# MDIL-SNU/SevenNet

Hardware: NVIDIA H100
Metric: atom_updates_per_sec (higher is better)
Workload: dtype f32

## Files before the change

sevenn_b200/csrc/common.cuh:

```cuda
#pragma once
#include <cuda_runtime.h>
#include <cstdint>
#include <cstdio>

#include "vec_ops.cuh"

namespace s7b {

constexpr float kSiluNorm = 1.6791767923989418f;
constexpr int kMaxPaths = 12;
constexpr int kMaxL = 4;

S7B_HD float silu_n(float z) {
  const float s = 1.0f / (1.0f + expf(-z));
  return kSiluNorm * z * s;
}
S7B_HD float dsilu_n(float z) {
  const float s = 1.0f / (1.0f + expf(-z));
  return kSiluNorm * s * (1.0f + z * (1.0f - s));
}

struct ConvRole {
  int x_off;
  int mul;
  int tab_off;
  int w_off[kMaxPaths];
  int out_off[kMaxPaths];
  int out_stride[kMaxPaths];
  int ftab_off;
};

__host__ __device__ constexpr int y_stride(int ny) { return (ny - 1 + 3) / 4 * 4; }

constexpr int kConvWrongMul = 3;
constexpr int kConvNoPath = 4;

struct ConvArgs {
  const int* rowptr;
  const int4* rec;
  const float* Y;
  const float* x;
  const float4* table;
  const uint2* table23;
  const float* w;
  int n_begin, n_dst;
  int dim_x, dim_mid, w_numel;
  float inv_h;
  unsigned int* row_max;
  int rows_per_node;
  const float2* ftable;
  float ftab_inv_h;
  int ftab_knots;
};

struct ConvTangents {
  const float* x;
  const float* Y;
  const float* w;
};

}

#define S7B_CUDA_CHECK(expr)                                                            \
  do {                                                                                  \
    cudaError_t _e = (expr);                                                            \
    if (_e != cudaSuccess) {                                                            \
      s7b::set_error(__FILE__, __LINE__, cudaGetErrorString(_e));                       \
      return 1;                                                                         \
    }                                                                                   \
  } while (0)

namespace s7b {
void set_error(const char* file, int line, const char* msg);
}
```

sevenn_b200/csrc/conv_kernels.cuh:

```cuda
#pragma once
#include <cuda_fp16.h>

#include "common.cuh"
#include "generated/tp_kinds.cuh"
#include "tp_tangent.cuh"

namespace s7b {

constexpr int kConvWarpsPerBlock = 4;
constexpr int kConvMul[kMaxL] = {128, 64, 32, 32};
constexpr int kConvMaxMul = 1024;

template <int MUL>
__device__ __forceinline__ int conv_mul(const ConvRole& role) {
  if constexpr (MUL > 0) return MUL;
  else return role.mul;
}
#ifndef S7B_FWD_MINBLOCKS
#define S7B_FWD_MINBLOCKS 1
#endif
#define S7B_FWD_BOUNDS __launch_bounds__(32 * kConvWarpsPerBlock, S7B_FWD_MINBLOCKS)
#ifdef S7B_BWD_MINBLOCKS
#define S7B_BWD_BOUNDS __launch_bounds__(32 * kConvWarpsPerBlock, S7B_BWD_MINBLOCKS)
#else
#define S7B_BWD_BOUNDS __launch_bounds__(32 * kConvWarpsPerBlock, \
    (Kind::NY != 9 || (MUL == 0 && Kind::D1 > 1)) ? 2 : ((Kind::D1 == 3 || !NEED_DX) ? 4 : 3))
#endif
#ifndef S7B_COOP_REC
#define S7B_COOP_REC 1
#endif

constexpr float kValueTableMinR = 0.6f;

enum { kRecRaw = 0, kRecValue = 1, kRecCubicShort = 2 };
template <int MODE>
__device__ __forceinline__ int4 fwd_rec(const ConvArgs& a, int4 r, bool valid, bool& short_seen) {
  const float rr = __int_as_float(r.w);
  const bool is_short = valid && rr < kValueTableMinR;
  if (MODE == kRecValue) {
    short_seen = short_seen || is_short;
    const int k = is_short ? a.ftab_knots - 1 : min(max((int)(rr * a.ftab_inv_h), 0), a.ftab_knots - 1);
    const float t = is_short ? 1.0f : fminf(fmaxf(fmaf(rr, a.ftab_inv_h, -(float)k), 0.0f), 1.0f);
    return make_int4(r.x, k, __float_as_int(t), 0);
  }
  if (MODE == kRecCubicShort) return make_int4(r.x, is_short ? r.y : ~r.y, r.z, 0);
  return r;
}

template <int LPN>
struct EdgeRecs {
  int cx, cy, cz;
  __device__ __forceinline__ void fill(const ConvArgs& a, int e0, int len, int it, int sl) {
    const int ei = it + sl;
    int4 r = make_int4(0, 0, 0, 0);
    if (ei < len) r = __ldg(a.rec + (unsigned)(e0 + ei));
    cx = r.x; cy = r.y; cz = r.z;
  }
  template <int MODE>
  __device__ __forceinline__ void fill(const ConvArgs& a, int e0, int len, int it, int sl, bool& short_seen) {
    const int ei = it + sl;
    int4 r = make_int4(0, 0, 0, 0);
    if (ei < len) r = __ldg(a.rec + (unsigned)(e0 + ei));
    r = fwd_rec<MODE>(a, r, ei < len, short_seen);
    cx = r.x; cy = r.y; cz = r.z;
  }
  __device__ __forceinline__ int4 get(int it) const {
    const int l = it % LPN;
    return make_int4(__shfl_sync(0xffffffffu, cx, l, LPN), __shfl_sync(0xffffffffu, cy, l, LPN),
                     __shfl_sync(0xffffffffu, cz, l, LPN), 0);
  }
};

template <int M, int LPN>
__device__ __forceinline__ void group_reduce_multi(float (&v)[M], int sl) {
  static_assert((M == 8 || M == 16) && (LPN == 16 || LPN == 32) && M <= LPN, "unsupported reduction shape");
  int off = LPN / 2;
#pragma unroll
  for (int m = M / 2; m >= 1; m >>= 1, off >>= 1) {
    const bool up = (sl & off) != 0;
#pragma unroll
    for (int j = 0; j < m; ++j) {
      const float send = up ? v[j] : v[j + m];
      const float keep = up ? v[j + m] : v[j];
      v[j] = keep + __shfl_xor_sync(0xffffffffu, send, off);
    }
  }
#pragma unroll
  for (; off >= 1; off >>= 1) v[0] += __shfl_xor_sync(0xffffffffu, v[0], off);
}

template <int LPN>
__device__ __forceinline__ float group_sum(float v) {
#pragma unroll
  for (int off = LPN / 2; off >= 1; off >>= 1) v += __shfl_xor_sync(0xffffffffu, v, off);
  return v;
}

template <class Kind>
__device__ __forceinline__ void load_Y(const float* __restrict__ Yrow, float (&Y)[Kind::NY]) {
  Y[0] = 1.0f;
  constexpr int NQ = (Kind::NY - 1 + 3) / 4;
  const float4* p = reinterpret_cast<const float4*>(Yrow);
#pragma unroll
  for (int q = 0; q < NQ; ++q) {
    const float4 v = __ldg(p + q);
    if (4 * q + 1 < Kind::NY) Y[4 * q + 1] = v.x;
    if (4 * q + 2 < Kind::NY) Y[4 * q + 2] = v.y;
    if (4 * q + 3 < Kind::NY) Y[4 * q + 3] = v.z;
    if (4 * q + 4 < Kind::NY) Y[4 * q + 4] = v.w;
  }
}

__device__ __forceinline__ size_t row_offset(int i, int stride) { return (size_t)(unsigned)i * (unsigned)stride; }

__device__ __forceinline__ float2 ldg2(const float* p) { return __ldg(reinterpret_cast<const float2*>(p)); }

template <class V> struct VT;
template <> struct VT<V2> {
  static constexpr int CH = 2;
  static __device__ __forceinline__ V2 zero() { return splat2(0.0f); }
  static __device__ __forceinline__ V2 load(const float* p) { return ldg2(p); }
  static __device__ __forceinline__ void store(float* p, V2 v) { *reinterpret_cast<float2*>(p) = v; }
// ... 13 lines not shown
  static constexpr int CH = 1;
  static __device__ __forceinline__ float zero() { return 0.0f; }
  static __device__ __forceinline__ float load(const float* p) { return __ldg(p); }
  static __device__ __forceinline__ void store(float* p, float v) { *p = v; }
  static __device__ __forceinline__ float hsum(float v) { return v; }
  static __device__ __forceinline__ float amax(float v) { return fabsf(v); }
  static __device__ __forceinline__ float val(const float2* p, bool odd) { return __ldg(reinterpret_cast<const float*>(p) + odd); }
  static __device__ __forceinline__ void coef(const float4* t01, const uint2* t23, bool odd, float& a0, float& a1, float& a2, float& a3) {
    const float4 c01 = __ldg(t01);
    const uint2 c23 = __ldg(t23);
    const float2 h2 = __half22float2(*reinterpret_cast<const __half2*>(&c23.x));
    const float2 h3 = __half22float2(*reinterpret_cast<const __half2*>(&c23.y));
    a0 = odd ? c01.y : c01.x;
    a1 = odd ? c01.w : c01.z;
    a2 = odd ? h2.y : h2.x;
    a3 = odd ? h3.y : h3.x;
  }
};

template <int NV, int LPN, int CH>
struct LaneMap {
  int n, sl, uc0, e0, len, nmax;
  bool node_ok;
  __device__ __forceinline__ LaneMap(const ConvArgs& a) {
    constexpr int GPW = 32 / LPN;
    const int lane = threadIdx.x & 31;
    sl = lane % LPN;
    n = a.n_begin + (blockIdx.x * kConvWarpsPerBlock + (threadIdx.x >> 5)) * GPW + lane / LPN;
    node_ok = n < a.n_dst;
    uc0 = blockIdx.y * (CH * LPN * NV) + CH * sl;
    e0 = 0;
    len = 0;
    if (node_ok) {
      e0 = __ldg(a.rowptr + n);
      len = __ldg(a.rowptr + n + 1) - e0;
    }
    nmax = len;
    if (GPW > 1) nmax = max(len, __shfl_xor_sync(0xffffffffu, len, 16));
  }
};

template <class Kind, int MUL, int NV, int LPN, bool TABLE, class V, int MODE>
__device__ __forceinline__ void conv_fwd_edges(const ConvArgs& a, const ConvRole& role,
                                               const LaneMap<NV, LPN, VT<V>::CH>& m,
                                               V (&acc)[NV][Kind::NACC], bool& short_seen) {
  constexpr int CH = VT<V>::CH;
  const int mul = conv_mul<MUL>(role);
  const unsigned xlane = role.x_off + m.uc0;
  const unsigned tlane = (MODE == kRecCubicShort ? role.tab_off : role.ftab_off) + (m.uc0 >> 1);
  const bool odd = (m.uc0 & 1) != 0;
  EdgeRecs<LPN> recs;
  for (int it = 0; it < m.nmax; ++it) {
    const bool valid = (LPN == 32) || (it < m.len);
    const int e = valid ? m.e0 + it : 0;
#if S7B_COOP_REC
    if (it % LPN == 0) recs.template fill<MODE>(a, m.e0, m.len, it, m.sl, short_seen);
    const int4 rec = recs.get(it);
#else
    const int4 rec = fwd_rec<MODE>(a, __ldg(a.rec + e), valid, short_seen);
#endif
    float Y[Kind::NY];
    load_Y<Kind>(a.Y + row_offset(e, y_stride(Kind::NY)), Y);
    const float* __restrict__ xrow = a.x + (row_offset(rec.x, a.dim_x) + xlane);
    const bool take = MODE != kRecCubicShort || rec.y >= 0;
    const int k = take ? rec.y : ~rec.y;
    const unsigned ti = tlane + k * (Kind::NPATH * mul / 2);
    const float2* __restrict__ v0 = a.ftable + ti;
    const float2* __restrict__ v1 = v0 + Kind::NPATH * mul / 2;
    const float tt = __int_as_float(rec.z);
#pragma unroll
    for (int c = 0; c < NV; ++c) {
      const int u = CH * LPN * c;
      V x[Kind::D1], w[Kind::NPATH];
#pragma unroll
      for (int i = 0; i < Kind::D1; ++i) x[i] = VT<V>::load(xrow + i * mul + u);
#pragma unroll
      for (int p = 0; p < Kind::NPATH; ++p) {
        if (MODE == kRecValue) {
          const V w0 = VT<V>::val(v0 + (p * (mul / 2) + u / 2), odd);
          const V w1 = VT<V>::val(v1 + (p * (mul / 2) + u / 2), odd);
          w[p] = fma_(tt, w1, fma_(-tt, w0, w0));
        } else if (MODE == kRecCubicShort) {
          V a0, a1, a2, a3;
          VT<V>::coef(a.table + ti + (p * (mul / 2) + u / 2), a.table23 + ti + (p * (mul / 2) + u / 2), odd, a0, a1, a2, a3);
          w[p] = take ? fma_(tt, fma_(tt, fma_(tt, a3, a2), a1), a0) : VT<V>::zero();
        } else {
          w[p] = VT<V>::load(a.w + (size_t)e * a.w_numel + role.w_off[p] + m.uc0 + u);
        }
        if (LPN != 32 && !valid) w[p] = VT<V>::zero();
      }
      Kind::fwd(x, Y, w, acc[c]);
    }
  }
}

template <class Kind, int MUL, int NV, int LPN, bool TABLE, class V>
__global__ void S7B_FWD_BOUNDS
conv_fwd_kernel(const ConvArgs a, const ConvRole role, float* __restrict__ out) {
  constexpr int CH = VT<V>::CH;
  static_assert(MUL % (CH * LPN * NV) == 0, "channels must fill whole lane groups");
  const LaneMap<NV, LPN, CH> m(a);
  if (m.nmax == 0 && !m.node_ok) return;

  V acc[NV][Kind::NACC];
#pragma unroll
  for (int c = 0; c < NV; ++c)
#pragma unroll
    for (int q = 0; q < Kind::NACC; ++q) acc[c][q] = VT<V>::zero();

  bool short_seen = false;
  conv_fwd_edges<Kind, MUL, NV, LPN, TABLE, V, TABLE ? kRecValue : kRecRaw>(a, role, m, acc, short_seen);
// ... 22 lines not shown
      }
    }
  }
  if (!m.node_ok) return;
  float* __restrict__ orow = out + (size_t)m.n * a.dim_mid;
#pragma unroll
  for (int c = 0; c < NV; ++c) {
    const int u = m.uc0 + CH * LPN * c;
#pragma unroll
    for (int p = 0; p < Kind::NPATH; ++p) {
#pragma unroll
      for (int k = 0; k < 2 * Kind::path_l3(p) + 1; ++k)
        VT<V>::store(orow + role.out_off[p] + k * role.out_stride[p] + u, acc[c][Kind::acc_off(p) + k]);
    }
  }
}

template <class Kind, int MUL, int NV, int LPN, bool TABLE, bool NEED_DX>
__global__ void S7B_BWD_BOUNDS
conv_bwd_kernel(const ConvArgs a, const ConvRole role, const float* __restrict__ gout,
                float* __restrict__ dx, float* __restrict__ dY_acc, float* __restrict__ dEdr_acc,
                float* __restrict__ dw) {
  static_assert(MUL % (2 * LPN * NV) == 0, "channels must fill whole lane groups");
  const int mul = conv_mul<MUL>(role);
  const bool SPLIT = (MUL > 0) ? (MUL > 2 * LPN * NV) : (gridDim.y > 1);
  const LaneMap<NV, LPN, 2> m(a);
  if (m.nmax == 0) return;

  V2 ga[NV][Kind::NACC];
  {
    const float* __restrict__ grow = gout + (size_t)(m.node_ok ? m.n : 0) * a.dim_mid;
#pragma unroll
    for (int c = 0; c < NV; ++c) {
      const int u = m.uc0 + 2 * LPN * c;
#pragma unroll
      for (int p = 0; p < Kind::NPATH; ++p)
#pragma unroll
        for (int k = 0; k < 2 * Kind::path_l3(p) + 1; ++k)
          ga[c][Kind::acc_off(p) + k] = ldg2(grow + role.out_off[p] + k * role.out_stride[p] + u);
    }
  }

  constexpr int NR = (Kind::NY <= 9) ? 8 : 16;
  constexpr bool RIDE = TABLE && (Kind::NY - 1 < NR);
  constexpr int PER = LPN / NR;
  const int idx = (m.sl / PER) % NR;
  const bool is_dY = idx + 1 < Kind::NY;
  const bool writer = (m.sl % PER) == 0 && (is_dY || (RIDE && idx == NR - 1));
  const unsigned xlane = role.x_off + m.uc0;
  const unsigned tlane = role.tab_off + (m.uc0 >> 1);
  EdgeRecs<LPN> recs;
  for (int it = 0; it < m.nmax; ++it) {
    const bool valid = (LPN == 32) || (it < m.len);
    const int e = valid ? m.e0 + it : 0;
#if S7B_COOP_REC
    if (it % LPN == 0) recs.fill(a, m.e0, m.len, it, m.sl);
    const int4 rec = recs.get(it);
#else
    const int4 rec = __ldg(a.rec + e);
#endif
    float Y[Kind::NY];
    load_Y<Kind>(a.Y + row_offset(e, y_stride(Kind::NY)), Y);
    const size_t xo = row_offset(rec.x, a.dim_x) + xlane;
    const unsigned ti = tlane + rec.y * (Kind::NPATH * mul / 2);
    const float4* __restrict__ k01 = a.table + ti;
    const uint2* __restrict__ k23 = a.table23 + ti;
    const float tt = __int_as_float(rec.z);
    V2 dY[Kind::NY];
#pragma unroll
    for (int j = 0; j < Kind::NY; ++j) dY[j] = splat2(0.0f);
    V2 dEdr2 = splat2(0.0f);
#pragma unroll
    for (int c = 0; c < NV; ++c) {
      const int u = 2 * LPN * c;
      V2 x[Kind::D1], w[Kind::NPATH], wd[Kind::NPATH], dwv[Kind::NPATH], dxv[Kind::D1];
#pragma unroll
      for (int i = 0; i < Kind::D1; ++i) x[i] = ldg2(a.x + xo + (i * mul + u));
#pragma unroll
      for (int p = 0; p < Kind::NPATH; ++p) {
        if (TABLE) {
          const float4 c01 = __ldg(k01 + (p * (mul / 2) + u / 2));
          const uint2 c23 = __ldg(k23 + (p * (mul / 2) + u / 2));
          const V2 a0 = make_float2(c01.x, c01.y), a1 = make_float2(c01.z, c01.w);
          const V2 a2 = __half22float2(*reinterpret_cast<const __half2*>(&c23.x));
          const V2 a3 = __half22float2(*reinterpret_cast<const __half2*>(&c23.y));
          w[p] = fma_(tt, fma_(tt, fma_(tt, a3, a2), a1), a0);
          wd[p] = mul_(fma_(tt, fma_(3.0f * tt, a3, mul_(a2, 2.0f)), a1), a.inv_h);
        } else {
          w[p] = ldg2(a.w + (size_t)e * a.w_numel + role.w_off[p] + m.uc0 + u);
        }
      }
      Kind::bwd(x, Y, w, ga[c], dwv, dxv, dY);
      if (valid) {
#pragma unroll
        for (int p = 0; p < Kind::NPATH; ++p) {
          if (TABLE) dEdr2 = fma_(dwv[p], wd[p], dEdr2);
          else *reinterpret_cast<float2*>(dw + (size_t)e * a.w_numel + role.w_off[p] + m.uc0 + u) = dwv[p];
        }
        if (NEED_DX) {
#pragma unroll
          for (int i = 0; i < Kind::D1; ++i)
            atomicAdd(reinterpret_cast<float2*>(dx + xo + (i * mul + u)), dxv[i]);
        }
      }
    }
    const float dEdr = dEdr2.x + dEdr2.y;
    float red[NR];
#pragma unroll
    for (int j = 0; j < NR; ++j) red[j] = (j + 1 < Kind::NY) ? dY[j + 1].x + dY[j + 1].y : 0.0f;
    if (RIDE) red[NR - 1] = dEdr;
    group_reduce_multi<NR, LPN>(red, m.sl);
    if (valid && writer) {
      float* dst = is_dY ? dY_acc + row_offset(e, y_stride(Kind::NY)) + idx : dEdr_acc + e;
      if (SPLIT) atomicAdd(dst, red[0]);
      else *dst += red[0];
    }
    if (TABLE && !RIDE) {
      const float s = group_sum<LPN>(dEdr);
      if (valid && m.sl == 0) {
        if (SPLIT) atomicAdd(dEdr_acc + e, s);
        else dEdr_acc[e] += s;
      }
    }
  }
}

template <class Kind, int NV, int LPN>
__global__ void S7B_FWD_BOUNDS
conv_jvp_kernel(const ConvArgs a, const ConvRole role, const ConvTangents tan, float* __restrict__ out) {
  const LaneMap<NV, LPN, 2> m(a);
  if (m.nmax == 0 && !m.node_ok) return;
  const int mul = role.mul;
  const bool hx = tan.x != nullptr, hY = tan.Y != nullptr, hw = tan.w != nullptr;

  V2 acc[NV][Kind::NACC];
#pragma unroll
  for (int c = 0; c < NV; ++c)
#pragma unroll
    for (int q = 0; q < Kind::NACC; ++q) acc[c][q] = splat2(0.0f);

  const unsigned xlane = role.x_off + m.uc0;
  EdgeRecs<LPN> recs;
  for (int it = 0; it < m.nmax; ++it) {
    const bool valid = (LPN == 32) || (it < m.len);
    const int e = valid ? m.e0 + it : 0;
    if (it % LPN == 0) recs.fill(a, m.e0, m.len, it, m.sl);
    const int4 rec = recs.get(it);
    float Y[Kind::NY], tY[Kind::NY];
    load_Y<Kind>(a.Y + row_offset(e, y_stride(Kind::NY)), Y);
    if (hY) load_Y<Kind>(tan.Y + row_offset(e, y_stride(Kind::NY)), tY);
    const size_t xo = row_offset(rec.x, a.dim_x) + xlane;
    const size_t wo = (size_t)e * a.w_numel + m.uc0;
#pragma unroll
    for (int c = 0; c < NV; ++c) {
      const int u = 2 * LPN * c;
      V2 x[Kind::D1], tx[Kind::D1], w[Kind::NPATH], tw[Kind::NPATH];
#pragma unroll
      for (int i = 0; i < Kind::D1; ++i) {
        x[i] = ldg2(a.x + xo + (i * mul + u));
        if (hx) tx[i] = ldg2(tan.x + xo + (i * mul + u));
      }
#pragma unroll
      for (int p = 0; p < Kind::NPATH; ++p) {
        w[p] = ldg2(a.w + wo + (role.w_off[p] + u));
        if (hw) tw[p] = ldg2(tan.w + wo + (role.w_off[p] + u));
        if (LPN != 32 && !valid) w[p] = tw[p] = splat2(0.0f);
      }
      TPTangent<Kind>::jvp(x, Y, w, tx, tY, tw, hx, hY, hw, acc[c]);
    }
  }
  if (!m.node_ok) return;
  float* __restrict__ orow = out + (size_t)m.n * a.dim_mid;
#pragma unroll
  for (int c = 0; c < NV; ++c) {
    const int u = m.uc0 + 2 * LPN * c;
#pragma unroll
    for (int p = 0; p < Kind::NPATH; ++p) {
#pragma unroll
      for (int k = 0; k < 2 * Kind::path_l3(p) + 1; ++k)
        VT<V2>::store(orow + role.out_off[p] + k * role.out_stride[p] + u, acc[c][Kind::acc_off(p) + k]);
    }
  }
}

enum { kTanDw = 1, kTanDx = 2, kTanDY = 4 };
template <class Kind, int NV, int LPN, int OUT>
__device__ __forceinline__ void conv_bwd_tangent_edges(const ConvArgs& a, const ConvRole& role, const ConvTangents& tan,
                                                       const LaneMap<NV, LPN, 2>& m, const V2 (&ga)[NV][Kind::NACC],
                                                       float* __restrict__ dx, float* __restrict__ dY_acc,
                                                       float* __restrict__ dw) {
  constexpr bool DW = (OUT & kTanDw) != 0, DX = (OUT & kTanDx) != 0, DY = (OUT & kTanDY) != 0;
  const int mul = role.mul;
  const bool SPLIT = gridDim.y > 1;
  const bool hx = tan.x != nullptr, hY = tan.Y != nullptr, hw = tan.w != nullptr;
  const bool need_dx = DX && (hY || hw);
  constexpr int NR = (Kind::NY <= 9) ? 8 : 16;
  constexpr int PER = LPN / NR;
  const int idx = (m.sl / PER) % NR;
  const bool writer = (m.sl % PER) == 0 && idx + 1 < Kind::NY;
  const unsigned xlane = role.x_off + m.uc0;
  EdgeRecs<LPN> recs;
  for (int it = 0; it < m.nmax; ++it) {
    const bool valid = (LPN == 32) || (it < m.len);
    const int e = valid ? m.e0 + it : 0;
    if (it % LPN == 0) recs.fill(a, m.e0, m.len, it, m.sl);
    const int4 rec = recs.get(it);
    float Y[Kind::NY], tY[Kind::NY];
    load_Y<Kind>(a.Y + row_offset(e, y_stride(Kind::NY)), Y);
    if (hY && (DW || DX)) load_Y<Kind>(tan.Y + row_offset(e, y_stride(Kind::NY)), tY);
    const size_t xo = row_offset(rec.x, a.dim_x) + xlane;
    const size_t wo = (size_t)e * a.w_numel + m.uc0;
    V2 dY[Kind::NY];
#pragma unroll
    for (int j = 0; j < Kind::NY; ++j) dY[j] = splat2(0.0f);
#pragma unroll
    for (int c = 0; c < NV; ++c) {
      const int u = 2 * LPN * c;
      V2 x[Kind::D1], tx[Kind::D1], w[Kind::NPATH], tw[Kind::NPATH], dwv[Kind::NPATH], dxv[Kind::D1];
#pragma unroll
      for (int i = 0; i < Kind::D1; ++i) {
        x[i] = ldg2(a.x + xo + (i * mul + u));
        if (hx && (DW || DY)) tx[i] = ldg2(tan.x + xo + (i * mul + u));
      }
#pragma unroll
      for (int p = 0; p < Kind::NPATH; ++p) {
        w[p] = ldg2(a.w + wo + (role.w_off[p] + u));
        if (hw && (DX || DY)) tw[p] = ldg2(tan.w + wo + (role.w_off[p] + u));
      }
      TPTangent<Kind>::template bwd<DW, DX, DY>(x, Y, w, ga[c], tx, tY, tw, hx, hY, hw, dwv, dxv, dY);
      if (valid) {
        if (DW) {
#pragma unroll
          for (int p = 0; p < Kind::NPATH; ++p)
            *reinterpret_cast<float2*>(dw + wo + (role.w_off[p] + u)) = dwv[p];
        }
        if (need_dx) {
#pragma unroll
          for (int i = 0; i < Kind::D1; ++i)
            atomicAdd(reinterpret_cast<float2*>(dx + xo + (i * mul + u)), dxv[i]);
        }
      }
    }
    if (DY) {
      float red[NR];
#pragma unroll
      for (int j = 0; j < NR; ++j) red[j] = (j + 1 < Kind::NY) ? dY[j + 1].x + dY[j + 1].y : 0.0f;
      group_reduce_multi<NR, LPN>(red, m.sl);
      if (valid && writer) {
        float* dst = dY_acc + row_offset(e, y_stride(Kind::NY)) + idx;
        if (SPLIT) atomicAdd(dst, red[0]);
        else *dst += red[0];
      }
    }
  }
}

template <class Kind>
constexpr bool tangent_walk_per_output() { return Kind::NACC * (Kind::D1 + Kind::NY) > 400; }

// ... 31 lines not shown
```

sevenn_b200/csrc/edge_kernels.cuh:

```cuda
#pragma once
#include "common.cuh"
#include "generated/sh.cuh"

namespace s7b {

struct RadialDesc {
  float cutoff;
  int cutoff_fn;
  float cutoff_on;
  int poly_p;
  int n_basis;
  float coeffs[8];
  float inv_h;
  int knots;
};

S7B_HD void envelope(const RadialDesc& d, float r, float& env, float& denv) {
  if (d.cutoff_fn == 0) {
    if (r < d.cutoff_on) { env = 1.0f; denv = 0.0f; return; }
    const float r2 = r * r, on2 = d.cutoff_on * d.cutoff_on, c2 = d.cutoff * d.cutoff;
    const float den = (c2 - on2) * (c2 - on2) * (c2 - on2);
    const float a = c2 - r2, b = c2 + 2.0f * r2 - 3.0f * on2;
    env = a * a * b / den;
    denv = (-4.0f * r * a * b + 4.0f * r * a * a) / den;
  } else {
    const float p = (float)d.poly_p;
    const float x = r / d.cutoff;
    float xp = 1.0f;
    for (int i = 0; i < d.poly_p - 1; ++i) xp *= x;
    const float c0 = (p + 1.0f) * (p + 2.0f) * 0.5f, c1 = p * (p + 2.0f), c2 = p * (p + 1.0f) * 0.5f;
    env = 1.0f - xp * x * (c0 - c1 * x + c2 * x * x);
    denv = -xp * (c0 * p - c1 * (p + 1.0f) * x + c2 * (p + 2.0f) * x * x) / d.cutoff;
  }
}

template <int LMAX>
__global__ void edge_fwd_kernel(const RadialDesc rd, const float* __restrict__ edge_vec,
                                const int* __restrict__ src, const int64_t* __restrict__ n_edges_p, int ny_stride,
                                int4* __restrict__ rec, float* __restrict__ Yout,
                                float* __restrict__ rlen, float* __restrict__ emb) {
  const int64_t e = (int64_t)blockIdx.x * blockDim.x + threadIdx.x;
  if (e >= *n_edges_p) return;
  const float vx = edge_vec[3 * e], vy = edge_vec[3 * e + 1], vz = edge_vec[3 * e + 2];
  const float r = sqrtf(vx * vx + vy * vy + vz * vz);
  const float ir = r > 0.0f ? 1.0f / r : 0.0f;
  float Y[SH<LMAX>::NY];
  SH<LMAX>::eval(vx * ir, vy * ir, vz * ir, Y);
  float* yrow = Yout + e * ny_stride;
#pragma unroll
  for (int j = 1; j < SH<LMAX>::NY; ++j) yrow[j - 1] = Y[j];
  for (int j = SH<LMAX>::NY - 1; j < ny_stride; ++j) yrow[j] = 0.0f;
  const float s = r * rd.inv_h;
  int tk = (int)s;
  tk = tk < 0 ? 0 : (tk > rd.knots - 1 ? rd.knots - 1 : tk);
  const float tt = fminf(fmaxf(s - (float)tk, 0.0f), 1.0f);
  rec[e] = make_int4(__ldg(src + e), tk, __float_as_int(tt), __float_as_int(r));
  rlen[e] = r;
  if (emb != nullptr) {
    float env, denv;
    envelope(rd, r, env, denv);
    const float pre = 2.0f / rd.cutoff;
    for (int b = 0; b < rd.n_basis; ++b) emb[e * rd.n_basis + b] = pre * sinf(rd.coeffs[b] * r) * ir * env;
  }
}

template <int LMAX>
__global__ void edge_bwd_kernel(const RadialDesc rd, const float* __restrict__ edge_vec,
                                const int64_t* __restrict__ n_edges_p, int64_t part_stride, int ny_stride, int n_part,
// ... 94 lines not shown
```

sevenn_b200/csrc/engine.cu:

```cuda
#include <algorithm>
#include <cstdlib>
#include <cstring>
#include <functional>
#include <map>
#include <string>
#include <vector>

#include "../../include/sevenn_b200.h"
#include "common.cuh"
#include "conv_kernels.cuh"
#include "edge_kernels.cuh"
#include "hvp_kernels.cuh"
#include "neighbor.cuh"
#include "node_kernels.cuh"
#include "tc_gemm.cuh"

namespace s7b {

static thread_local std::string g_error;
static int64_t g_launches = 0;
extern int64_t g_conv_launches;

void set_error(const char* file, int line, const char* msg) {
  char buf[512];
// ... 137 lines not shown
struct LayerParams {
  NodeLinear si1, si1T, sc, scT, si2, si2T;
  DevBuf table, table23, table_fwd;
  int ftab_knots = 0;
  DevBuf mlp[3], mlpT[3];
  void release() {
    for (NodeLinear* s : {&si1, &si1T, &sc, &scT, &si2, &si2T})
      for (DevBuf* b : {&s->w, &s->tc.q, &s->tc.fb}) b->release();
    for (DevBuf* b : {&table, &table23, &table_fwd, &mlp[0], &mlp[1], &mlp[2], &mlpT[0], &mlpT[1], &mlpT[2]}) b->release();
  }
};

struct HvpBufs {
  DevBuf dvec, dr, dY, gY, dgY, ar, dar, fneg, virial;
  DevBuf emb3, hA, hB, w3, dw, aw, daw1, daw2;
  DevBuf ah, dah, ag, dag, amid, damid, dmid, ax, dax, th;
  DevBuf atom_ptr1, sys_energy, dvir2;
  std::vector<DevBuf> tx, tg;
  RowExp re;
  void release() {
    for (DevBuf* b : {&dvec, &dr, &dY, &gY, &dgY, &ar, &dar, &fneg, &virial, &emb3, &hA, &hB, &w3, &dw, &aw, &daw1, &daw2,
                      &ah, &dah, &ag, &dag, &amid, &damid, &dmid, &ax, &dax, &th, &atom_ptr1, &sys_energy, &dvir2, &re.buf})
      b->release();
    for (auto* v : {&tx, &tg})
      for (DevBuf& b : *v) b.release();
  }
};

struct GlobalParams {
  DevBuf embed_x0, embed_g0, readout, readout_lo, scale, shift;
  void release() {
    for (DevBuf* b : {&embed_x0, &embed_g0, &readout, &readout_lo, &scale, &shift}) b->release();
  }
};

}

using namespace s7b;

struct S7bEngine {
  S7bModelDesc desc;
  std::vector<LayerCfg> layers;
  std::vector<LayerParams> layer_params;
  GlobalParams global_params;
  RadialDesc radial;
  bool radial_ready = false;
  int ny_stride = 8;
  int n_nodes = 0, n_local = 0, n_interior = 0;
  int64_t n_edges = 0;
  const int* d_species = nullptr;
  const int* d_rowptr = nullptr;
  const int* d_src = nullptr;
  const float* d_edge_vec = nullptr;
  DevBuf rec, Y, rlen, emb, dY_acc, dEdr_acc, demb_acc, fedge;
  std::vector<DevBuf> x, g, wbuf, z1, z2, h1, h2;
  DevBuf mid, h, dh, dg, dx, dwbuf, tmpA, tmpB;
  RowExp re_mid, re_h, re_dg, re_dx;
  DevBuf energy, atomic_energy, atomic_energy64, forces, virial, atomic_virial;
  bool want_atomic_virial = false;
  DevBuf hs_species, hs_rowptr, hs_src, hs_vec, hs_centre, hs_flag;
  DevBuf nl_pos, nl_wrapped, nl_key, nl_key_sorted, nl_idx, nl_idx_sorted, nl_bin_start, nl_count, nl_tmp, nl_centres;
  DevBuf nl_species, nl_grids, nl_atom_ptr, nl_bin_off, nl_lohi, nl_sys, nl_total;
  std::vector<NLGrid> nl_grids_host;
  std::vector<int> nl_bin_off_host;
  int nl_n_centres = 0;
  int64_t nl_n_edges = 0;
  int n_systems = 0;
  bool species_sc = false;
  DevBuf seg_perm, seg;
  DevBuf sys_atom_ptr;
  Profiler prof;
  cudaStream_t side[kMaxL] = {nullptr, nullptr, nullptr, nullptr};
  cudaEvent_t ev_fork = nullptr, ev_join[kMaxL] = {nullptr, nullptr, nullptr, nullptr};
  bool concurrent = true;
  int64_t E_cap = 0;
  DevBuf d_nE;
  cudaGraphExec_t gexec = nullptr;
  cudaStream_t gstream = nullptr;
  cudaEvent_t g_in = nullptr, g_out = nullptr;
  std::vector<int64_t> g_key;
  int64_t g_launches_per_replay = 0;
  int64_t g_captures = 0, g_replays = 0;
  struct StageGraph {
    cudaGraphExec_t exec = nullptr;
    std::vector<int64_t> key;
    int64_t launches = 0, replays_since_capture = 0;
    int thrash = 0;
  };
  std::map<int, StageGraph> stage_graphs;
  bool capturing = false;
  int64_t sg_captures = 0, sg_replays = 0;
  bool hvp_ready = false;
  HvpBufs hv;
};

struct S7bConvPlan {
  LayerCfg cfg;
  int lmax_filter = 0;
  int ny_stride = 8;
};

namespace s7b {

static int irreps_dim(const int* muls, int n_l) {
  int d = 0;
  for (int l = 0; l < n_l; ++l) d += (2 * l + 1) * muls[l];
  return d;
// ... 682 lines not shown
    P.si2 = {&L.mid, &L.g, L.g.n_l};
    P.si2T = {&L.g, &L.mid, L.g.n_l};
  }
  e->ny_stride = y_stride((d->lmax_filter + 1) * (d->lmax_filter + 1));
  e->x.resize(T);
  e->g.resize(T);
  e->wbuf.resize(T);
  e->z1.resize(T);
  e->z2.resize(T);
  e->h1.resize(T);
  e->h2.resize(T);
  memset(&e->radial, 0, sizeof(e->radial));
  e->radial.cutoff = d->cutoff;
  e->radial.cutoff_fn = d->cutoff_fn;
  e->radial.cutoff_on = d->cutoff_on;
  e->radial.poly_p = d->poly_p;
  e->radial.n_basis = d->n_basis;
  e->radial.knots = d->table_knots > 0 ? d->table_knots : 1;
  e->radial.inv_h = d->table_knots > 0 ? (float)d->table_knots / d->cutoff : 1.0f;
  e->want_atomic_virial = g_opt_atomic_virial != 0;
  for (int i = 1; i < kMaxL; ++i) {
    if (cudaStreamCreateWithFlags(&e->side[i], cudaStreamNonBlocking) != cudaSuccess ||
        cudaEventCreateWithFlags(&e->ev_join[i], cudaEventDisableTiming) != cudaSuccess) {
      delete e;
      return fail("cannot create side streams");
    }
  }
  if (cudaEventCreateWithFlags(&e->ev_fork, cudaEventDisableTiming) != cudaSuccess) {
    delete e;
    return fail("cannot create events");
  }
  *out = e;
  return 0;
}

void s7b_engine_destroy(S7bEngine* e) {
  if (!e) return;
  for (int i = 1; i < kMaxL; ++i) {
    if (e->side[i]) cudaStreamDestroy(e->side[i]);
    if (e->ev_join[i]) cudaEventDestroy(e->ev_join[i]);
  }
  if (e->ev_fork) cudaEventDestroy(e->ev_fork);
  if (e->gexec) cudaGraphExecDestroy(e->gexec);
  for (auto& kv : e->stage_graphs) if (kv.second.exec) cudaGraphExecDestroy(kv.second.exec);
  if (e->gstream) cudaStreamDestroy(e->gstream);
  if (e->g_in) cudaEventDestroy(e->g_in);
  if (e->g_out) cudaEventDestroy(e->g_out);
  e->d_nE.release();
  e->global_params.release();
  for (LayerParams& P : e->layer_params) P.release();
  for (RowExp* r : {&e->re_mid, &e->re_h, &e->re_dg, &e->re_dx}) r->buf.release();
  e->seg_perm.release();
  e->seg.release();
  DevBuf* bufs[] = {&e->rec, &e->Y, &e->rlen, &e->emb, &e->dY_acc, &e->dEdr_acc, &e->demb_acc, &e->fedge,
                    &e->mid, &e->h, &e->dh, &e->dg, &e->dx, &e->dwbuf, &e->tmpA, &e->tmpB, &e->energy,
                    &e->atomic_energy, &e->forces, &e->virial, &e->atomic_virial, &e->hs_species, &e->hs_rowptr, &e->hs_src,
                    &e->hs_vec, &e->hs_centre, &e->hs_flag, &e->nl_pos, &e->nl_wrapped, &e->nl_key, &e->nl_key_sorted,
                    &e->nl_idx, &e->nl_idx_sorted, &e->nl_bin_start, &e->nl_count, &e->nl_tmp, &e->nl_centres,
                    &e->nl_species, &e->nl_grids, &e->nl_atom_ptr, &e->nl_bin_off, &e->nl_lohi, &e->nl_sys, &e->nl_total,
                    &e->sys_atom_ptr, &e->atomic_energy64};
  for (DevBuf* b : bufs) b->release();
  for (auto* v : {&e->x, &e->g, &e->wbuf, &e->z1, &e->z2, &e->h1, &e->h2})
    for (auto& b : *v) b.release();
  e->hv.release();
  delete e;
}

int s7b_engine_set_atomic_virial(S7bEngine* e, int enable) {
  if (!e) return fail("null engine");
  if (e->want_atomic_virial != (enable != 0)) ++g_alloc_gen;
  e->want_atomic_virial = enable != 0;
  return 0;
}

static int upload(DevBuf& dst, const float* host, size_t numel, const std::string& what) {
  if (dst.ensure(numel * sizeof(float))) return fail("cudaMalloc failed for " + what);
  S7B_CUDA_CHECK(cudaMemcpy(dst.p, host, numel * sizeof(float), cudaMemcpyHostToDevice));
  return 0;
}

int s7b_engine_set_param(S7bEngine* e, const char* name, int layer, const float* host, size_t numel) {
  if (!e || !name || !host) return fail("null argument");
  const std::string nm(name);
  if (!(e->desc.table_knots > 0 && nm.compare(0, 3, "mlp") == 0)) e->hvp_ready = false;
  const int T = e->desc.n_layers, S = e->desc.num_species, nb = e->desc.n_basis;
  const std::string what = (layer >= 0 ? "layer " + std::to_string(layer) + ": " : std::string()) + "parameter " + nm;
  auto bad_size = [&](size_t expect) {
    return numel == expect ? 0 : fail(what + " has " + std::to_string(numel) + " values, expected " + std::to_string(expect));
  };
  GlobalParams& G = e->global_params;
  const LayerCfg &L0 = e->layers[0], &Lz = e->layers[T - 1];
  const struct { const char* name; DevBuf* buf; size_t numel; } globals[] = {
      {"embed_x0", &G.embed_x0, (size_t)S * L0.x.dim}, {"embed_g0", &G.embed_g0, (size_t)S * L0.g.dim},
      {"readout", &G.readout, (size_t)Lz.dim_h},       {"readout_lo", &G.readout_lo, (size_t)Lz.dim_h},
      {"scale", &G.scale, (size_t)S},                  {"shift", &G.shift, (size_t)S},
      {"bessel", nullptr, (size_t)nb}};
  for (const auto& g : globals) {
    if (nm != g.name) continue;
    if (layer >= 0) return fail(what + " is global: its layer must be negative");
    if (bad_size(g.numel)) return 1;
    if (g.buf) return upload(*g.buf, host, numel, what);
    for (int b = 0; b < nb; ++b) e->radial.coeffs[b] = host[b];
    e->radial_ready = true;
    return 0;
  }
  static const std::pair<const char*, NodeLinear LayerParams::*> linears[] = {
      {"si1", &LayerParams::si1}, {"si1T", &LayerParams::si1T}, {"sc", &LayerParams::sc}, {"scT", &LayerParams::scT},
// ... 47 lines not shown
      return upload(dst, img.data(), numel, what);
    }
    const size_t rows = numel / (size_t)L.W;
    if (numel % (size_t)L.W != 0 || rows < 2 || rows * (size_t)L.W / 2 > (size_t)INT32_MAX)
      return fail(what + " has " + std::to_string(numel) + " values, expected (knots + 1) x " + std::to_string(L.W) +
                  " with at least one interval");
    for (size_t c = 0; c < (size_t)L.W; ++c)
      if (host[(rows - 1) * L.W + c] != 0.0f) return fail(what + ": the last knot (r = cutoff) must be 0");
    const std::vector<float> img = role_table_images(L, (int)rows, host, 2, off);
    if (upload(dst, img.data(), numel, what)) return 1;
    for (int l1 = 0; l1 < L.x.n_l; ++l1) L.roles[l1].ftab_off = off[l1];
    P.ftab_knots = (int)rows - 1;
    return 0;
  }
  const int j = mlp % 3;
  const int dims[4] = {nb, e->desc.radial_hidden[0], e->desc.radial_hidden[1], L.W};
  if (bad_size((size_t)dims[j] * dims[j + 1])) return 1;
  return upload(mlp < 3 ? P.mlp[j] : P.mlpT[j], host, numel, what);
}

int s7b_engine_set_graph(S7bEngine* e, int32_t n_nodes, int32_t n_local, int64_t n_edges,
                         const int32_t* d_species, const int32_t* d_rowptr, const int32_t* d_src,
                         const float* d_edge_vec, void* stream) {
  if (!e) return fail("null engine");
  if (n_local < 0 || n_nodes < n_local || n_edges < 0) return fail("bad graph sizes");
  if (n_edges >= ((int64_t)1 << 31)) return fail("more than 2^31-1 edges per GPU are not supported");
  e->hvp_ready = false;
  e->n_nodes = n_nodes;
  e->n_local = n_local;
  e->n_interior = n_local;
  e->n_edges = n_edges;
  e->d_species = d_species;
  e->d_rowptr = d_rowptr;
  e->d_src = d_src;
  e->d_edge_vec = d_edge_vec;
  e->n_systems = 0;
  const bool table = e->desc.table_knots > 0;
  if (n_edges > e->E_cap || 2 * n_edges < e->E_cap)
    e->E_cap = (n_edges + n_edges / 32 + 1024) / 1024 * 1024;
  if (e->d_nE.ensure(sizeof(int64_t))) return fail("cudaMalloc failed");
  set_i64_kernel<<<1, 1, 0, reinterpret_cast<cudaStream_t>(stream)>>>(e->d_nE.as<int64_t>(), n_edges);
  S7B_LAUNCH_CHECK();
  const size_t E = (size_t)e->E_cap, Nn = (size_t)std::max(n_nodes, 1), Nl = (size_t)std::max(n_local, 1);
  const int T = e->desc.n_layers;
  int rc = 0;
  rc |= e->rec.ensure(E * sizeof(int4));
  rc |= e->Y.ensure(E * e->ny_stride * sizeof(float));
  rc |= e->rlen.ensure(E * sizeof(float));
  int max_lx = 0;
  for (auto& L : e->layers) max_lx = std::max(max_lx, L.x.n_l);
  rc |= e->dY_acc.ensure((size_t)max_lx * E * e->ny_stride * sizeof(float));
  rc |= e->dEdr_acc.ensure((size_t)max_lx * E * sizeof(float));
  rc |= e->fedge.ensure(E * 3 * sizeof(float));
  size_t max_mid = 0, max_h = 0, max_g = 0, max_x = 0, max_W = 0;
  for (int t = 0; t < T; ++t) {
    const LayerCfg& L = e->layers[t];
    rc |= e->x[t].ensure(Nn * L.x.dim * sizeof(float));
    rc |= e->g[t].ensure(Nl * L.g.dim * sizeof(float));
    max_mid = std::max(max_mid, (size_t)L.mid.dim);
    max_h = std::max(max_h, (size_t)L.dim_h);
    max_g = std::max(max_g, (size_t)L.g.dim);
    max_x = std::max(max_x, (size_t)L.x.dim);
    max_W = std::max(max_W, (size_t)L.W);
    if (!table) {
      const int h0 = e->desc.radial_hidden[0], h1 = e->desc.radial_hidden[1];
      rc |= e->wbuf[t].ensure(E * L.W * sizeof(float));
      rc |= e->z1[t].ensure(E * h0 * sizeof(float));
      rc |= e->h1[t].ensure(E * h0 * sizeof(float));
      rc |= e->z2[t].ensure(E * h1 * sizeof(float));
      rc |= e->h2[t].ensure(E * h1 * sizeof(float));
    }
  }
  if (!table) {
    rc |= e->emb.ensure(E * e->desc.n_basis * sizeof(float));
    rc |= e->demb_acc.ensure(E * e->desc.n_basis * sizeof(float));
    rc |= e->dwbuf.ensure(E * max_W * sizeof(float));
    const size_t hh = (size_t)std::max(e->desc.radial_hidden[0], e->desc.radial_hidden[1]);
    rc |= e->tmpA.ensure(E * hh * sizeof(float));
    rc |= e->tmpB.ensure(E * hh * sizeof(float));
  }
  rc |= e->mid.ensure(Nl * max_mid * sizeof(float));
  rc |= e->h.ensure(Nl * std::max(max_h, max_x) * sizeof(float));
  rc |= e->dh.ensure(Nl * std::max(max_h, max_x) * sizeof(float));
  rc |= e->dg.ensure(Nl * max_g * sizeof(float));
  rc |= e->dx.ensure(Nn * max_x * sizeof(float));
  if (e->species_sc) rc |= e->seg_perm.ensure(Nl * sizeof(int));
  for (RowExp* r : {&e->re_mid, &e->re_h, &e->re_dg, &e->re_dx}) rc |= r->buf.ensure(Nn * 16 * sizeof(int));
  rc |= e->energy.ensure(sizeof(double));
  rc |= e->virial.ensure(6 * sizeof(double));
  rc |= e->atomic_energy.ensure(Nl * sizeof(float));
  rc |= e->atomic_energy64.ensure(Nl * sizeof(double));
  rc |= e->forces.ensure(Nn * 3 * sizeof(float));
  if (e->want_atomic_virial) rc |= e->atomic_virial.ensure(Nn * 6 * sizeof(float));
  if (rc) return fail("cudaMalloc failed while sizing step buffers");
  return 0;
}

int s7b_engine_set_interior(S7bEngine* e, int32_t n_interior) {
  if (!e) return fail("null engine");
  if (n_interior < 0 || n_interior > e->n_local) return fail("n_interior out of range");
  e->n_interior = n_interior;
  return 0;
}

static ConvArgs make_conv_args(const S7bEngine* e, int t, const float* x) {
  const LayerCfg& L = e->layers[t];
  const LayerParams& P = e->layer_params[t];
  ConvArgs a;
  memset(&a, 0, sizeof(a));
  a.rowptr = e->d_rowptr;
  a.rec = e->rec.as<int4>();
  a.Y = e->Y.as<float>();
  a.x = x;
  a.table = P.table.as<const float4>();
  a.table23 = P.table23.as<const uint2>();
  a.w = e->desc.table_knots > 0 ? nullptr : e->wbuf[t].as<float>();
  a.n_dst = e->n_local;
  a.dim_x = L.x.dim;
  a.dim_mid = L.mid.dim;
  a.w_numel = L.W;
  a.inv_h = e->radial.inv_h;
  a.ftable = P.table_fwd.as<const float2>();
  a.ftab_knots = P.ftab_knots;
  a.ftab_inv_h = P.ftab_knots > 0 ? (float)P.ftab_knots / e->desc.cutoff : 0.0f;
  return a;
}

static int grid1d(size_t total, int block) {
  size_t g = (total + block - 1) / block;
  if (g > 132 * 64) g = 132 * 64;
  if (g < 1) g = 1;
  return (int)g;
}

static int require(const void* p, const char* what) {
  if (p) return 0;
  return fail(std::string("missing parameter: ") + what);
}

static int run_stage_impl(S7bEngine* e, int stage, int t, void* stream) {
  cudaStream_t st = reinterpret_cast<cudaStream_t>(stream);
  const int T = e->desc.n_layers;
  const int Nn = e->n_nodes, Nl = e->n_local;
  const int64_t E = e->n_edges;
  const int64_t Ecap = e->E_cap;
  const int64_t* nE = e->d_nE.as<int64_t>();
  const bool table = e->desc.table_knots > 0;
  const int LF = e->desc.lmax_filter;
  if (!e->radial_ready) return fail("parameter 'bessel' was not set");

  switch (stage) {
    case S7B_STAGE_FWD_BEGIN: {
      if (E > 0) {
        const int blk = 256;
        const int grd = (int)((Ecap + blk - 1) / blk);
        float* emb = table ? nullptr : e->emb.as<float>();
        ProfScope ps(e->prof, st, "edge_fwd");
        if (LF == 1) edge_fwd_kernel<1><<<grd, blk, 0, st>>>(e->radial, e->d_edge_vec, e->d_src, nE, e->ny_stride, e->rec.as<int4>(), e->Y.as<float>(), e->rlen.as<float>(), emb);
        else if (LF == 2) edge_fwd_kernel<2><<<grd, blk, 0, st>>>(e->radial, e->d_edge_vec, e->d_src, nE, e->ny_stride, e->rec.as<int4>(), e->Y.as<float>(), e->rlen.as<float>(), emb);
        else edge_fwd_kernel<3><<<grd, blk, 0, st>>>(e->radial, e->d_edge_vec, e->d_src, nE, e->ny_stride, e->rec.as<int4>(), e->Y.as<float>(), e->rlen.as<float>(), emb);
        S7B_LAUNCH_CHECK();
        int max_lx = 0;
        for (auto& L : e->layers) max_lx = std::max(max_lx, L.x.n_l);
        S7B_CUDA_CHECK(cudaMemsetAsync(e->dY_acc.p, 0, (size_t)max_lx * Ecap * e->ny_stride * sizeof(float), st));
        S7B_CUDA_CHECK(cudaMemsetAsync(e->dEdr_acc.p, 0, (size_t)max_lx * Ecap * sizeof(float), st));
// ... 535 lines not shown
  return 0;
}

int s7b_engine_set_profiling(S7bEngine* e, int enable) {
  if (!e) return fail("null engine");
  e->prof.clear();
  e->prof.enabled = enable != 0;
  return 0;
}

int s7b_engine_profile_count(S7bEngine* e) {
  if (!e) return 0;
  e->prof.collect();
  return (int)e->prof.totals.size();
}

int s7b_engine_profile_entry(S7bEngine* e, int index, char* name, size_t name_len, double* total_ms,
                             int64_t* calls) {
  if (!e) return fail("null engine");
  e->prof.collect();
  if (index < 0 || index >= (int)e->prof.totals.size()) return fail("profile index out of range");
  auto it = e->prof.totals.begin();
  std::advance(it, index);
  if (name && name_len > 0) snprintf(name, name_len, "%s", it->first.c_str());
  if (total_ms) *total_ms = it->second.first;
  if (calls) *calls = it->second.second;
  return 0;
}

void* s7b_engine_buffer(S7bEngine* e, const char* name, int layer, size_t* numel) {
  if (!e || !name) return nullptr;
  const std::string nm(name);
  const int T = e->desc.n_layers;
  size_t n = 0;
  void* p = nullptr;
  auto in_range = [&](int t) { return t >= 0 && t < T; };
  if (nm == "x" && in_range(layer)) { p = e->x[layer].p; n = (size_t)e->n_nodes * e->layers[layer].x.dim; }
  else if (nm == "gate_in" && in_range(layer)) { p = e->g[layer].p; n = (size_t)e->n_local * e->layers[layer].g.dim; }
  else if (nm == "weight" && in_range(layer)) { p = e->wbuf[layer].p; n = (size_t)e->n_edges * e->layers[layer].W; }
  else if (nm == "dx" && in_range(layer)) { p = e->dx.p; n = (size_t)e->n_nodes * e->layers[layer].x.dim; }
  else if (nm == "dg" && in_range(layer)) { p = e->dg.p; n = (size_t)e->n_local * e->layers[layer].g.dim; }
  else if (nm == "mid" && in_range(layer)) { p = e->mid.p; n = (size_t)e->n_local * e->layers[layer].mid.dim; }
  else if (nm == "h" && in_range(layer)) { p = e->h.p; n = (size_t)e->n_local * e->layers[layer].dim_h; }
  else if (nm == "dh" && in_range(layer)) { p = e->dh.p; n = (size_t)e->n_local * e->layers[layer].x.dim; }
  else if (nm == "energy") { p = e->energy.p; n = 1; }
  else if (nm == "virial") { p = e->virial.p; n = 6; }
  else if (nm == "atomic_energy") { p = e->atomic_energy.p; n = (size_t)e->n_local; }
  else if (nm == "atomic_energy_f64") { p = e->atomic_energy64.p; n = (size_t)e->n_local; }
  else if (nm == "atomic_virial" && e->want_atomic_virial) { p = e->atomic_virial.p; n = (size_t)e->n_nodes * 6; }
  else if (nm == "forces") { p = e->forces.p; n = (size_t)e->n_nodes * 3; }
  else if (nm == "edge_force") { p = e->fedge.p; n = (size_t)e->n_edges * 3; }
  else if (nm == "edge_Y") { p = e->Y.p; n = (size_t)e->n_edges * e->ny_stride; }
  else if (nm == "edge_rec") { p = e->rec.p; n = (size_t)e->n_edges * 4; }
  else if (nm == "graph_rowptr") { p = (void*)e->d_rowptr; n = (size_t)e->n_local + 1; }
  else if (nm == "graph_src") { p = (void*)e->d_src; n = (size_t)e->n_edges; }
  else if (nm == "graph_edge_vec") { p = (void*)e->d_edge_vec; n = (size_t)e->n_edges * 3; }
  else if (nm == "nl_rowptr") { p = e->hs_rowptr.p; n = (size_t)e->nl_n_centres + 1; }
  else if (nm == "nl_src") { p = e->hs_src.p; n = (size_t)e->nl_n_edges; }
  else if (nm == "nl_vec") { p = e->hs_vec.p; n = (size_t)e->nl_n_edges * 3; }
  else if (nm == "edge_len") { p = e->rlen.p; n = (size_t)e->n_edges; }
  else if (nm == "edge_emb") { p = e->emb.p; n = (size_t)e->n_edges * e->desc.n_basis; }
  else if (nm == "dY_acc" || nm == "dEdr_acc") {
    int max_lx = 0;
    for (auto& L : e->layers) max_lx = std::max(max_lx, L.x.n_l);
    const int part = layer < 0 ? 0 : layer;
    const bool dY = nm == "dY_acc";
    float* base = dY ? e->dY_acc.as<float>() : e->dEdr_acc.as<float>();
    if (base && layer >= -1 && part < max_lx) {
      const size_t row = dY ? (size_t)e->ny_stride : 1;
      p = base + (size_t)part * e->E_cap * row;
      n = (size_t)e->n_edges * row;
    }
  }
  if (numel) *numel = n;
  return p;
}

int s7b_engine_compute_host(S7bEngine* e, int32_t n_nodes, int64_t n_edges, const int32_t* species,
                            const int32_t* edge_centre, const int32_t* edge_neighbour,
                            const float* edge_vec, double* energy, float* atomic_energy, float* forces,
                            double* virial, void* stream) {
  if (!e) return fail("null engine");
  if (n_nodes < 0 || n_edges < 0) return fail("bad sizes");
  if (n_nodes > 0 && !species) return fail("null species");
  if (n_edges > 0 && (!edge_centre || !edge_neighbour || !edge_vec)) return fail("null edge arrays");
  cudaStream_t st = reinterpret_cast<cudaStream_t>(stream);
  const size_t E = (size_t)std::max<int64_t>(n_edges, 1), N = (size_t)std::max(n_nodes, 1);
  if (e->hs_species.ensure(N * sizeof(int)) || e->hs_rowptr.ensure((N + 1) * sizeof(int)) ||
      e->hs_src.ensure(E * sizeof(int)) || e->hs_vec.ensure(E * 3 * sizeof(float)) ||
      e->hs_centre.ensure(E * sizeof(int)) || e->hs_flag.ensure(sizeof(int)))
    return fail("cudaMalloc failed for staging buffers");
  if (n_nodes > 0) S7B_CUDA_CHECK(cudaMemcpyAsync(e->hs_species.p, species, (size_t)n_nodes * sizeof(int), cudaMemcpyHostToDevice, st));
  S7B_CUDA_CHECK(cudaMemsetAsync(e->hs_flag.p, 0, sizeof(int), st));
  if (n_edges > 0) {
    S7B_CUDA_CHECK(cudaMemcpyAsync(e->hs_centre.p, edge_centre, (size_t)n_edges * sizeof(int), cudaMemcpyHostToDevice, st));
    S7B_CUDA_CHECK(cudaMemcpyAsync(e->hs_src.p, edge_neighbour, (size_t)n_edges * sizeof(int), cudaMemcpyHostToDevice, st));
    S7B_CUDA_CHECK(cudaMemcpyAsync(e->hs_vec.p, edge_vec, (size_t)n_edges * 3 * sizeof(float), cudaMemcpyHostToDevice, st));
  }
  {
    const int64_t nthreads = n_edges + 1;
    csr_from_sorted_kernel<<<(int)((nthreads + 255) / 256), 256, 0, st>>>(e->hs_centre.as<int>(), e->hs_src.as<int>(), n_edges, n_nodes, e->hs_rowptr.as<int>(), e->hs_flag.as<int>());
    S7B_LAUNCH_CHECK();
    int flag = 0;
    S7B_CUDA_CHECK(cudaMemcpyAsync(&flag, e->hs_flag.p, sizeof(int), cudaMemcpyDeviceToHost, st));
    S7B_CUDA_CHECK(cudaStreamSynchronize(st));
    if (flag & 1) return fail("edges must be sorted by centre and centres must be < n_nodes");
// ... 509 lines not shown
```

Baseline: 1.847 million.

## Process each node's edges in distance-sorted order via a per-row permutation

Adds a warp-per-row kernel that ranks every node's incoming edges by squared length, then source index, and writes a permutation into a new edge_order buffer. The convolution forward, backward and tangent kernels now read each edge id through this permutation instead of using contiguous edge indices. The likely aim is to make neighbouring iterations hit nearby radial table knots and to group short edges, improving cache locality and reducing divergence. In exchange it adds a quadratic-per-row sort kernel each step, an extra indirection load per edge, and scattered rather than sequential Y and rec accesses.

```diff
diff --git a/sevenn_b200/csrc/common.cuh b/sevenn_b200/csrc/common.cuh
--- a/sevenn_b200/csrc/common.cuh
+++ b/sevenn_b200/csrc/common.cuh
@@ -51,6 +51,7 @@
   const float2* ftable;
   float ftab_inv_h;
   int ftab_knots;
+  const int* order;
 };
 
 struct ConvTangents {
diff --git a/sevenn_b200/csrc/conv_kernels.cuh b/sevenn_b200/csrc/conv_kernels.cuh
--- a/sevenn_b200/csrc/conv_kernels.cuh
+++ b/sevenn_b200/csrc/conv_kernels.cuh
@@ -47,27 +47,37 @@
   return r;
 }
 
+__device__ __forceinline__ int edge_slot(const ConvArgs& a, int i) { return a.order ? __ldg(a.order + i) : i; }
+
 template <int LPN>
 struct EdgeRecs {
-  int cx, cy, cz;
+  int cx, cy, cz, ce;
   __device__ __forceinline__ void fill(const ConvArgs& a, int e0, int len, int it, int sl) {
     const int ei = it + sl;
     int4 r = make_int4(0, 0, 0, 0);
-    if (ei < len) r = __ldg(a.rec + (unsigned)(e0 + ei));
-    cx = r.x; cy = r.y; cz = r.z;
+    int e = 0;
+    if (ei < len) {
+      e = edge_slot(a, e0 + ei);
+      r = __ldg(a.rec + (unsigned)e);
+    }
+    cx = r.x; cy = r.y; cz = r.z; ce = e;
   }
   template <int MODE>
   __device__ __forceinline__ void fill(const ConvArgs& a, int e0, int len, int it, int sl, bool& short_seen) {
     const int ei = it + sl;
     int4 r = make_int4(0, 0, 0, 0);
-    if (ei < len) r = __ldg(a.rec + (unsigned)(e0 + ei));
+    int e = 0;
+    if (ei < len) {
+      e = edge_slot(a, e0 + ei);
+      r = __ldg(a.rec + (unsigned)e);
+    }
     r = fwd_rec<MODE>(a, r, ei < len, short_seen);
-    cx = r.x; cy = r.y; cz = r.z;
+    cx = r.x; cy = r.y; cz = r.z; ce = e;
   }
   __device__ __forceinline__ int4 get(int it) const {
     const int l = it % LPN;
     return make_int4(__shfl_sync(0xffffffffu, cx, l, LPN), __shfl_sync(0xffffffffu, cy, l, LPN),
-                     __shfl_sync(0xffffffffu, cz, l, LPN), 0);
+                     __shfl_sync(0xffffffffu, cz, l, LPN), __shfl_sync(0xffffffffu, ce, l, LPN));
   }
 };
 
@@ -187,11 +197,12 @@
   EdgeRecs<LPN> recs;
   for (int it = 0; it < m.nmax; ++it) {
     const bool valid = (LPN == 32) || (it < m.len);
-    const int e = valid ? m.e0 + it : 0;
 #if S7B_COOP_REC
     if (it % LPN == 0) recs.template fill<MODE>(a, m.e0, m.len, it, m.sl, short_seen);
     const int4 rec = recs.get(it);
+    const int e = rec.w;
 #else
+    const int e = valid ? edge_slot(a, m.e0 + it) : 0;
     const int4 rec = fwd_rec<MODE>(a, __ldg(a.rec + e), valid, short_seen);
 #endif
     float Y[Kind::NY];
@@ -320,11 +331,12 @@
   EdgeRecs<LPN> recs;
   for (int it = 0; it < m.nmax; ++it) {
     const bool valid = (LPN == 32) || (it < m.len);
-    const int e = valid ? m.e0 + it : 0;
 #if S7B_COOP_REC
     if (it % LPN == 0) recs.fill(a, m.e0, m.len, it, m.sl);
     const int4 rec = recs.get(it);
+    const int e = rec.w;
 #else
+    const int e = valid ? edge_slot(a, m.e0 + it) : 0;
     const int4 rec = __ldg(a.rec + e);
 #endif
     float Y[Kind::NY];
@@ -411,9 +423,9 @@
   EdgeRecs<LPN> recs;
   for (int it = 0; it < m.nmax; ++it) {
     const bool valid = (LPN == 32) || (it < m.len);
-    const int e = valid ? m.e0 + it : 0;
     if (it % LPN == 0) recs.fill(a, m.e0, m.len, it, m.sl);
     const int4 rec = recs.get(it);
+    const int e = rec.w;
     float Y[Kind::NY], tY[Kind::NY];
     load_Y<Kind>(a.Y + row_offset(e, y_stride(Kind::NY)), Y);
     if (hY) load_Y<Kind>(tan.Y + row_offset(e, y_stride(Kind::NY)), tY);
@@ -470,9 +482,9 @@
   EdgeRecs<LPN> recs;
   for (int it = 0; it < m.nmax; ++it) {
     const bool valid = (LPN == 32) || (it < m.len);
-    const int e = valid ? m.e0 + it : 0;
     if (it % LPN == 0) recs.fill(a, m.e0, m.len, it, m.sl);
     const int4 rec = recs.get(it);
+    const int e = rec.w;
     float Y[Kind::NY], tY[Kind::NY];
     load_Y<Kind>(a.Y + row_offset(e, y_stride(Kind::NY)), Y);
     if (hY && (DW || DX)) load_Y<Kind>(tan.Y + row_offset(e, y_stride(Kind::NY)), tY);
diff --git a/sevenn_b200/csrc/edge_kernels.cuh b/sevenn_b200/csrc/edge_kernels.cuh
--- a/sevenn_b200/csrc/edge_kernels.cuh
+++ b/sevenn_b200/csrc/edge_kernels.cuh
@@ -14,6 +14,37 @@
   float inv_h;
   int knots;
 };
+
+__global__ void edge_order_kernel(const int* __restrict__ rowptr, const int* __restrict__ src,
+                                  const float* __restrict__ edge_vec, int n_rows, int* __restrict__ order) {
+  const int row = (int)((blockIdx.x * (size_t)blockDim.x + threadIdx.x) >> 5);
+  const int lane = threadIdx.x & 31;
+  if (row >= n_rows) return;
+  const int e0 = rowptr[row], len = rowptr[row + 1] - e0;
+  auto key = [&](int i, unsigned& r2, int& s) {
+    const float* v = edge_vec + 3 * (size_t)(e0 + i);
+    r2 = __float_as_uint(v[0] * v[0] + v[1] * v[1] + v[2] * v[2]);
+    s = src[e0 + i];
+  };
+  for (int ci = 0; ci < len; ci += 32) {
+    const int i = ci + lane;
+    unsigned ri = 0;
+    int si = 0, rank = 0;
+    if (i < len) key(i, ri, si);
+    for (int cj = 0; cj < len; cj += 32) {
+      unsigned rj = 0;
+      int sj = 0;
+      if (cj + lane < len) key(cj + lane, rj, sj);
+      const int nj = min(32, len - cj);
+      for (int k = 0; k < nj; ++k) {
+        const unsigned rk = __shfl_sync(0xffffffffu, rj, k);
+        const int sk = __shfl_sync(0xffffffffu, sj, k), j = cj + k;
+        rank += rk < ri || (rk == ri && (sk < si || (sk == si && j < i)));
+      }
+    }
+    if (i < len) order[e0 + rank] = e0 + i;
+  }
+}
 
 S7B_HD void envelope(const RadialDesc& d, float r, float& env, float& denv) {
   if (d.cutoff_fn == 0) {
diff --git a/sevenn_b200/csrc/engine.cu b/sevenn_b200/csrc/engine.cu
--- a/sevenn_b200/csrc/engine.cu
+++ b/sevenn_b200/csrc/engine.cu
@@ -213,7 +213,7 @@
   const int* d_rowptr = nullptr;
   const int* d_src = nullptr;
   const float* d_edge_vec = nullptr;
-  DevBuf rec, Y, rlen, emb, dY_acc, dEdr_acc, demb_acc, fedge;
+  DevBuf rec, Y, rlen, emb, dY_acc, dEdr_acc, demb_acc, fedge, edge_order;
   std::vector<DevBuf> x, g, wbuf, z1, z2, h1, h2;
   DevBuf mid, h, dh, dg, dx, dwbuf, tmpA, tmpB;
   RowExp re_mid, re_h, re_dg, re_dx;
@@ -1002,7 +1002,7 @@
   for (RowExp* r : {&e->re_mid, &e->re_h, &e->re_dg, &e->re_dx}) r->buf.release();
   e->seg_perm.release();
   e->seg.release();
-  DevBuf* bufs[] = {&e->rec, &e->Y, &e->rlen, &e->emb, &e->dY_acc, &e->dEdr_acc, &e->demb_acc, &e->fedge,
+  DevBuf* bufs[] = {&e->rec, &e->Y, &e->rlen, &e->emb, &e->dY_acc, &e->dEdr_acc, &e->demb_acc, &e->fedge, &e->edge_order,
                     &e->mid, &e->h, &e->dh, &e->dg, &e->dx, &e->dwbuf, &e->tmpA, &e->tmpB, &e->energy,
                     &e->atomic_energy, &e->forces, &e->virial, &e->atomic_virial, &e->hs_species, &e->hs_rowptr, &e->hs_src,
                     &e->hs_vec, &e->hs_centre, &e->hs_flag, &e->nl_pos, &e->nl_wrapped, &e->nl_key, &e->nl_key_sorted,
@@ -1156,6 +1156,7 @@
   rc |= e->dY_acc.ensure((size_t)max_lx * E * e->ny_stride * sizeof(float));
   rc |= e->dEdr_acc.ensure((size_t)max_lx * E * sizeof(float));
   rc |= e->fedge.ensure(E * 3 * sizeof(float));
+  rc |= e->edge_order.ensure(E * sizeof(int));
   size_t max_mid = 0, max_h = 0, max_g = 0, max_x = 0, max_W = 0;
   for (int t = 0; t < T; ++t) {
     const LayerCfg& L = e->layers[t];
@@ -1197,6 +1198,11 @@
   rc |= e->forces.ensure(Nn * 3 * sizeof(float));
   if (e->want_atomic_virial) rc |= e->atomic_virial.ensure(Nn * 6 * sizeof(float));
   if (rc) return fail("cudaMalloc failed while sizing step buffers");
+  if (n_local > 0 && n_edges > 0) {
+    edge_order_kernel<<<(int)(((int64_t)n_local * 32 + 255) / 256), 256, 0, reinterpret_cast<cudaStream_t>(stream)>>>(
+        d_rowptr, d_src, d_edge_vec, n_local, e->edge_order.as<int>());
+    S7B_LAUNCH_CHECK();
+  }
   return 0;
 }
 
@@ -1215,6 +1221,7 @@
   a.rowptr = e->d_rowptr;
   a.rec = e->rec.as<int4>();
   a.Y = e->Y.as<float>();
+  a.order = e->n_edges > 0 ? e->edge_order.as<int>() : nullptr;
   a.x = x;
   a.table = P.table.as<const float4>();
   a.table23 = P.table23.as<const uint2>();
@@ -1856,6 +1863,7 @@
   else if (nm == "edge_force") { p = e->fedge.p; n = (size_t)e->n_edges * 3; }
   else if (nm == "edge_Y") { p = e->Y.p; n = (size_t)e->n_edges * e->ny_stride; }
   else if (nm == "edge_rec") { p = e->rec.p; n = (size_t)e->n_edges * 4; }
+  else if (nm == "edge_order") { p = e->edge_order.p; n = (size_t)e->n_edges; }
   else if (nm == "graph_rowptr") { p = (void*)e->d_rowptr; n = (size_t)e->n_local + 1; }
   else if (nm == "graph_src") { p = (void*)e->d_src; n = (size_t)e->n_edges; }
   else if (nm == "graph_edge_vec") { p = (void*)e->d_edge_vec; n = (size_t)e->n_edges * 3; }
```

Result: faster. 1.874 million (median of 6 runs) (+1.4%).
